# maniacs-oss/shadow

Hardware: AMD Instinct MI355X
Metric: routing-table build GTEPS + packet-routes/sec at 1/2/4/8 MI355X (%HBM roofline) (higher is better)
Workload: dtype f64

## Files before the change

### shadow_amd/csrc/topo_build.cpp

```cpp
#include <dlfcn.h>

#include <cstdio>
#include <cstdlib>
#include <cstring>
#include <numeric>

#include "topo_host.h"

namespace shdtopo {

constexpr int64_t kTieProbeRows = 64;

int upload_layout(Topology* top, const std::vector<uint32_t>& src, const std::vector<uint32_t>& perm,
                  const std::vector<uint32_t>* bstart, double delta, hipStream_t st) {
    const int64_t rows = (int64_t)src.size();
    std::vector<uint32_t>& psrc = top->layPsrc;
    psrc.resize((size_t)rows);
    for (int64_t i = 0; i < rows; i++) psrc[(size_t)i] = src[(size_t)perm[(size_t)i]];
    HIPCHK(top->d_rowmap.ensure((size_t)rows));
    HIPCHK(top->d_bsrc.ensure((size_t)rows));
    HIPCHK(hipMemcpyAsync(top->d_rowmap.p, perm.data(), 4 * (size_t)rows, hipMemcpyHostToDevice, st));
    HIPCHK(hipMemcpyAsync(top->d_bsrc.p, psrc.data(), 4 * (size_t)rows, hipMemcpyHostToDevice, st));
    const std::vector<double> sh = source_shifts(top, psrc.data(), rows, delta);
    HIPCHK(top->d_srcsh.ensure((size_t)rows));
// ... 271 lines not shown
    }
    HIPCHK(hipEventRecord(top->ev0, st));
    HIPCHK(launch_pair_table_complete((int)A, c.row0, c.rows, top->d_elatAA.p, top->d_elossAA.p,
                                      top->d_vlossA.p, c.out_lr, c.out_hops, c.out_rowmin,
                                      top->d_stats.p, st));
    HIPCHK(hipEventRecord(top->ev1, st));
    return 0;
}

int upload_endpoints(Topology* top, RowsCall& c) {
    const int64_t rows = c.rows, A = c.A;
    c.src.resize((size_t)rows);
    c.tgt.resize((size_t)A);
    for (int64_t i = 0; i < rows; i++) c.src[(size_t)i] = (uint32_t)top->hp->inv[(size_t)top->attached[(size_t)(c.row0 + i)]];
    for (int64_t i = 0; i < A; i++) c.tgt[(size_t)i] = (uint32_t)top->hp->inv[(size_t)top->attached[(size_t)i]];
    HIPCHK(top->d_sources.ensure((size_t)rows));
    HIPCHK(top->d_targets.ensure((size_t)A));
    HIPCHK(hipMemcpyAsync(top->d_sources.p, c.src.data(), sizeof(uint32_t) * (size_t)rows, hipMemcpyHostToDevice, c.st));
    HIPCHK(hipMemcpyAsync(top->d_targets.p, c.tgt.data(), sizeof(uint32_t) * (size_t)A, hipMemcpyHostToDevice, c.st));
    c.K = batch_k(top);
    top->stats.peeled_targets = 0;
    HIPCHK(hipEventRecord(top->ev0, c.st));
    return 0;
}

int prepare_target_set(Topology* top, RowsCall& c) {
    hipStream_t st = c.st;
    const int64_t nadjk = (int64_t)(top->d_adjk.n / 4);
    const bool leaf = leaf_targets_on(top);
    if (leaf) {
        CHK(ensure_leaf_targets(top, c.tgt, top->d_targets.p, st));
        c.ws.tleaf = top->d_tleaf.p;
    }
    top->stats.peeled_targets = leaf ? top->leafPeeled : 0;
    if (!top->adjkPlain && (top->adjkTargets != c.tgt || top->adjkLeaf != leaf)) {
        HIPCHK(launch_kappa_copy(top->g.V, nadjk, hub_segs(top), top->d_rowptr.p, adj_out(top), top->d_pot.p,
                                 top->d_sptPar.p, top->d_adjk.p, top->d_kap.p,
                                 top->d_ksum.p, top->d_kap0.p, st));
        top->adjkPlain = true;
        top->adjkFlagged = false;
        top->adjkResorted = false;
        top->adjkLeaf = false;
        top->adjkTargets.clear();
    }
    if (!top->targetSkip || !top->adjkPlain) return 0;
    CHK(upload_target_bits(top, c.tgt, st));
    HIPCHK(hipEventRecord(top->evp0, st));
    const uint32_t* tbits = leaf ? top->d_tbitsEff.p : top->d_tbits.p;
    const uint32_t* dead = leaf ? top->d_dead.p : nullptr;
    HIPCHK(launch_mark_targets(top->d_adjk.p, nadjk, tbits, st));
    const int64_t V = top->g.V;
    const HubSegs hs = hub_segs(top);
    const int nit = std::max(0, top->targetKappa);
    HIPCHK(top->d_kfA.ensure(2 * (size_t)V));
    HIPCHK(top->d_kfB.ensure(2 * (size_t)V));
    HIPCHK(top->d_kfPart.ensure(std::max<size_t>(1, hs.nseg)));
    HIPCHK(top->d_kfChanged.ensure((size_t)nit + 1));
    if (!top->kfKapReady) {
        HIPCHK(top->d_kfKap.ensure((size_t)std::max<int64_t>(1, nadjk)));
        HIPCHK(launch_kfix_kap(adj_out(top), top->d_pot.p, nadjk, top->d_kfKap.p, st));
        top->kfKapReady = true;
    }
    HIPCHK(hipMemsetAsync(top->d_kfChanged.p, 0, sizeof(unsigned int) * ((size_t)nit + 1), st));
    HIPCHK(launch_kfix_step(top->d_rowptr.p, adj_out(top), top->d_kfKap.p, tbits,
                            nullptr, top->d_kfA.p, V, hs, top->d_kfPart.p,
                            top->d_kfChanged.p, st, dead));
// ... 856 lines not shown
```

### shadow_amd/csrc/topo_core.cpp

```cpp
#include <arpa/inet.h>

#include <condition_variable>
#include <cstdarg>
#include <cstdio>
#include <cstdlib>
#include <cstring>
#include <numeric>
#include <queue>
#include <unordered_set>

#include "topo_host.h"

extern "C" {
__attribute__((weak)) uint32_t address_toNetworkIP(Address* address);
__attribute__((weak)) double random_nextDouble(Random* random);
__attribute__((weak)) void worker_updateMinTimeJump(double minPathLatency);
__attribute__((weak)) void logging_log(const char* log_domain, int log_level, const char* fileName,
                                       const char* functionName, int lineNumber,
                                       const char* format, ...);
}
using namespace shdtopo;

namespace shdtopo {
namespace {
// ... 439 lines not shown
        hin.rows = H;
        hin.seg = iseg.p;
        hin.nseg = ns;
        hin.multi = imulti.p;
        hin.nmulti = nm;
        double pm = 0.0;
        HIPCHK(prep_tree(V, nadj, hin, top->d_rowptrIn.p, top->d_adj.p, top->d_aloss.p, top->d_pot.p,
                         top->d_sptPar.p, top->d_spt.p, &pm, st, kTreeParents));
        DevBuf<double> prev;
        HIPCHK(prev.ensure((size_t)V));
        int it2 = 0;
        HIPCHK(prep_h0_distances(V, top->d_rowptrIn.p, top->d_adj.p, prev.p, &it2, st));
        top->hp->potSrc.resize((size_t)V);
        HIPCHK(hipMemcpyAsync(top->hp->potSrc.data(), prev.p, 8 * (size_t)V, hipMemcpyDeviceToHost, st));
        HIPCHK(hipStreamSynchronize(st));
        double mx = 0.0;
        for (double x : top->hp->potSrc)
            if (std::isfinite(x) && x > mx) mx = x;
        top->hp->srcMax = mx;
    }
    step_done(4);
    HIPCHK(top->d_adjk.ensure(4 * (size_t)std::max<int64_t>(1, nadj)));
    HIPCHK(top->d_kap.ensure((size_t)std::max<int64_t>(1, nadj)));
    HIPCHK(top->d_ksum.ensure(kKProbes * (size_t)V));
    HIPCHK(top->d_kap0.ensure((size_t)V));
    HIPCHK(launch_kappa_copy(V, nadj, hub_segs(top), top->d_rowptr.p, adj_out(top), top->d_pot.p,
                             top->d_sptPar.p, top->d_adjk.p, top->d_kap.p, top->d_ksum.p,
                             top->d_kap0.p, st));
    top->adjkPlain = true;
    top->adjkFlagged = false;
    top->adjkLeaf = false;
    top->adjkTargets.clear();
    top->leafFor.clear();
    top->rowsSorted = true;
    HIPCHK(top->d_kfKap.ensure((size_t)std::max<int64_t>(1, nadj)));
    HIPCHK(launch_kfix_kap(adj_out(top), top->d_pot.p, nadj, top->d_kfKap.p, st));
    top->kfKapReady = true;
    step_done(5);
    {
        const auto tc = clk::now();
        top->hp->perm.resize((size_t)V);
        top->hp->inv.resize((size_t)V);
        top->hp->pot.resize((size_t)V);
        top->hp->sptPar.resize((size_t)V);
        HIPCHK(hipMemcpyAsync(top->hp->perm.data(), dperm.p, 4 * (size_t)V, hipMemcpyDeviceToHost, st));
        HIPCHK(hipMemcpyAsync(top->hp->inv.data(), dinv.p, 4 * (size_t)V, hipMemcpyDeviceToHost, st));
        HIPCHK(hipMemcpyAsync(top->hp->pot.data(), top->d_pot.p, 8 * (size_t)V, hipMemcpyDeviceToHost, st));
        HIPCHK(hipMemcpyAsync(top->hp->sptPar.data(), top->d_sptPar.p, 4 * (size_t)V, hipMemcpyDeviceToHost, st));
        HIPCHK(hipStreamSynchronize(st));
        copy_ms += ms_since(tc);
        const auto th = clk::now();
        tree_order(*top->hp);
        host_ms += ms_since(th);
    }
    step_done(6);
    MESSAGE("graph preparation: upload %.1f, relabel %.1f, rows %.1f, h0 distances %.1f (%d "
            "rounds), tree %.1f, kappa copy %.1f, host copies %.1f ms",
            top->stats.csr_step_ms[0], top->stats.csr_step_ms[1], top->stats.csr_step_ms[2],
            top->stats.csr_step_ms[3], iters, top->stats.csr_step_ms[4],
            top->stats.csr_step_ms[5], top->stats.csr_step_ms[6]);
    top->stats.csr_host_ms = host_ms;
    top->stats.csr_copy_ms = copy_ms;
    top->csrUploaded = true;
    return 0;
}

// ... 250 lines not shown
    std::vector<uint32_t> tb(words, 0u);
    for (uint32_t t : tgt) tb[t >> 5] |= 1u << (t & 31u);
    HIPCHK(top->d_tbits.ensure(words));
    HIPCHK(hipMemcpyAsync(top->d_tbits.p, tb.data(), 4 * words, hipMemcpyHostToDevice, st));
    HIPCHK(hipStreamSynchronize(st));
    return 0;
}

bool leaf_targets_on(const Topology* top) { return top->leafTargets && !top->isDirected; }

int ensure_leaf_targets(Topology* top, const std::vector<uint32_t>& tgt, const uint32_t* d_tgt,
                        hipStream_t st) {
    if (top->leafFor == tgt && top->d_tleaf.p) return 0;
    const size_t words = ((size_t)top->g.V + 31) / 32;
    const size_t A = tgt.size();
    std::vector<uint32_t> tb(words, 0u);
    for (uint32_t t : tgt) tb[t >> 5] |= 1u << (t & 31u);
    top->leafFor.clear();
    HIPCHK(top->d_tleaf.ensure(2 * std::max<size_t>(1, A)));
    HIPCHK(top->d_tbitsEff.ensure(words));
    HIPCHK(top->d_dead.ensure(words));
    HIPCHK(top->d_leafCount.ensure(1));
    HIPCHK(hipMemcpyAsync(top->d_tbitsEff.p, tb.data(), 4 * words, hipMemcpyHostToDevice, st));
    HIPCHK(hipMemsetAsync(top->d_dead.p, 0, 4 * words, st));
    HIPCHK(hipMemsetAsync(top->d_leafCount.p, 0, 4, st));
    HIPCHK(launch_leaf_targets(top->d_rowptr.p, top->d_adj.p, top->d_aloss.p, d_tgt, (int)A,
                               top->d_tleaf.p, top->d_tbitsEff.p, top->d_dead.p,
                               top->d_leafCount.p, st));
    uint32_t n = 0;
    HIPCHK(hipMemcpyAsync(&n, top->d_leafCount.p, 4, hipMemcpyDeviceToHost, st));
    HIPCHK(hipStreamSynchronize(st));
    top->leafPeeled = (int64_t)n;
    top->leafFor = tgt;
    return 0;
}

uint64_t compute_geometry(Topology* top) {
    std::vector<int32_t> vs;
    uint64_t sg;
    {
        std::shared_lock<std::shared_mutex> lk(top->ipMu);
        sg = top->setGen.load();
        if (top->geomInit && top->geomGen == top->ipGen) return sg;
        top->geomGen = top->ipGen;
        std::vector<int32_t> def(top->deferredOff.begin(), top->deferredOff.end());
        std::sort(def.begin(), def.end());
        vs.reserve(std::max<size_t>(top->A, 16));
        size_t k = 0;
        const uint32_t* on = top->hostsOn.data();
        for (int32_t v = 0; v < top->g.V; v++) {
            while (k < def.size() && def[k] < v) k++;
            if (on[v] || (k < def.size() && def[k] == v)) vs.push_back(v);
        }
    }
    if (top->geomInit && vs == top->attached) return sg;
    top->geomInit = true;
    top->attached = vs;
    top->A = (int64_t)vs.size();
    top->colOf.assign((size_t)top->g.V, -1);
    for (size_t i = 0; i < vs.size(); i++) top->colOf[(size_t)vs[i]] = (int32_t)i;
    top->colOfShared.reset();
    top->tableValid.store(false);
    if (top->isComplete) {
        auto pb = std::make_unique<Topology::PairBits>();
        pb->words = (size_t)((top->A * top->A + 63) / 64);
        pb->bits.reset(new std::atomic<uint64_t>[std::max<size_t>(1, pb->words)]);
// ... 518 lines not shown
            r = ensure_kprime_scratch(top, nullptr);
        if (!r) r = hipStreamSynchronize(top->stream) == hipSuccess ? 0 : -1;
        step(3);
        top->prepBgRc = r;
        top->prepBgMs = std::chrono::duration<double, std::milli>(std::chrono::steady_clock::now() - t0).count();
        if (onLoad) top->deviceUsed = used;
    });
}

void release_prepared(Topology* top) {
    release_workspace(top);
    for (auto* b : {&top->d_spt, &top->d_sptPar, &top->d_inv, &top->d_rowptr, &top->d_adj,
                    &top->d_adjo, &top->d_rowptrIn, &top->d_adjk})
        b->release();
    for (auto* b : {&top->d_elat, &top->d_eloss, &top->d_aloss, &top->d_vloss, &top->d_selfLat,
                    &top->d_selfLoss, &top->d_pot, &top->d_kfA, &top->d_kfB, &top->d_kfPart,
                    &top->d_kfKap})
        b->release();
    top->kfKapReady = false;
    top->kfFinal = nullptr;
    top->d_eu.release(); top->d_ev.release();
    top->d_kap.release(); top->d_ksum.release(); top->d_kap0.release();
    top->d_hseg.release(); top->d_hmulti.release(); top->d_kfChanged.release();
    top->d_kpKey.release(); top->d_kpIdx.release();
    top->d_kpRec.release(); top->d_kpTmp.release();
    top->d_kpBigPos.release(); top->d_kpBigRow.release(); top->d_kpBigVal.release();
    top->d_kpBigKey.release();
    top->kpBig = -1;
    top->hsegRows = top->hsegN = top->hmultiN = 0;
    top->csrUploaded = top->rowsSorted = false;
    top->adjkPlain = top->adjkFlagged = top->adjkResorted = top->adjkLeaf = false;
    top->adjkTargets.clear();
    top->leafFor.clear();
    top->ordUploaded = false;
    top->ordHp = nullptr;
    top->hp.reset();
}

void do_attach(Topology* top, uint32_t ip, int32_t v, uint64_t* bwDownOut, uint64_t* bwUpOut) {
    if (!top->firstAttachSet.load(std::memory_order_relaxed)) {
        std::unique_lock<std::shared_mutex> lk(top->ipMu);
        if (!top->firstAttachSet.load()) {
            top->firstAttachT = std::chrono::steady_clock::now();
            top->firstAttachSet.store(true);
        }
    }
    start_graph_prep(top, false);
    {
        std::unique_lock<std::shared_mutex> lk(top->ipMu);
        auto it = top->virtualIP.find(ip);
        const int32_t old = it == top->virtualIP.end() ? -1 : it->second;
        top->virtualIP[ip] = v;
        ip_tab_set(top, ip, v);
        top->ipGen++;
        if (old != v) {
            if (old >= 0) host_off(top, old);
            if (v >= 0) host_on(top, v);
        }
    }
    if (v >= 0) {
        if (bwUpOut) *bwUpOut = (uint64_t)top->g.vbwup[(size_t)v];
        if (bwDownOut) *bwDownOut = (uint64_t)top->g.vbwdown[(size_t)v];
    }
}

void do_detach(Topology* top, uint32_t ip) {
// ... 844 lines not shown
        const char* name;
        const void* host;
        const void* dev;
        size_t bytes;
        bool ok;
    };
    const Arr arrs[] = {
        {"perm", hp.perm.data(), nullptr, 4 * V, true},
        {"inv", hp.inv.data(), nullptr, 4 * V, true},
        {"rowptr", nullptr, top->d_rowptr.p, 4 * (V + 1), true},
        {"adj", nullptr, top->d_adj.p, 16 * nadj, true},
        {"aloss", nullptr, top->d_aloss.p, 8 * nadj, true},
        {"vloss", nullptr, top->d_vloss.p, 8 * V, true},
        {"self_lat", nullptr, top->d_selfLat.p, 8 * V, true},
        {"self_loss", nullptr, top->d_selfLoss.p, 8 * V, true},
        {"pot", hp.pot.data(), nullptr, 8 * V, true},
        {"pi_max", &hp.piMax, nullptr, 8, true},
        {"spt_parent", nullptr, top->d_sptPar.p, 4 * V, true},
        {"spt", nullptr, top->d_spt.p, 32 * V, true},
        {"adjk", nullptr, top->d_adjk.p, 16 * nadj, true},
        {"kap", nullptr, top->d_kap.p, 4 * nadj, true},
        {"ksum", nullptr, top->d_ksum.p, 4 * (size_t)kKProbes * V, true},
        {"kap0", nullptr, top->d_kap0.p, 4 * V, true},
        {"kf_kap", nullptr, top->d_kfKap.p, 8 * nadj, top->kfKapReady},
        {"hub_seg", nullptr, top->d_hseg.p, sizeof(uint2) * (size_t)top->hsegN, true},
        {"hub_multi", nullptr, top->d_hmulti.p, sizeof(uint4) * (size_t)top->hmultiN, true},
        {"rowptr_in", nullptr, top->d_rowptrIn.p, 4 * (V + 1), dir},
        {"adj_out", nullptr, top->d_adjo.p, 16 * nadj, dir},
        {"pot_src", hp.potSrc.data(), nullptr, 8 * V, dir && hp.potSrc.size() == V},
        {"tbits", nullptr, top->d_tbits.p, 4 * words, top->adjkFlagged && top->d_tbits.p},
        {"tbits_eff", nullptr, top->d_tbitsEff.p, 4 * words, leaf},
        {"dead", nullptr, top->d_dead.p, 4 * words, leaf},
        {"tleaf", nullptr, top->d_tleaf.p, 32 * top->leafFor.size(), leaf},
        {"kfix", nullptr, top->kfFinal, 16 * V, tprep},
        {"state", state, nullptr, sizeof state, true},
    };
    for (const Arr& a : arrs) {
        if (strcmp(a.name, name) != 0) continue;
        if (!a.ok) return -2;
        if (!out) return (int64_t)a.bytes;
        if (cap_bytes < (int64_t)a.bytes) return -3;
        if (a.bytes == 0) return 0;
        if (a.host) memcpy(out, a.host, a.bytes);
        else if (a.dev) HIPCHK(hipMemcpy(out, a.dev, a.bytes, hipMemcpyDeviceToHost));
        else return -2;
        return (int64_t)a.bytes;
    }
    return -1;
}

int shdtopo_export_graph(Topology* top, int32_t* eu, int32_t* ev, double* elat, double* eloss,
                         double* vloss) {
    if (!top) return -1;
    const HostGraph& g = top->g;
    const size_t E = (size_t)g.E, V = (size_t)g.V;
    if (eu) memcpy(eu, g.eu.data(), 4 * E);
    if (ev) memcpy(ev, g.ev.data(), 4 * E);
    if (elat) memcpy(elat, g.elat.data(), 8 * E);
    if (eloss) memcpy(eloss, g.eloss.data(), 8 * E);
    if (vloss) memcpy(vloss, g.vloss.data(), 8 * V);
    return 0;
}

int shdtopo_write_graphml(Topology* top, const char* path) {
    if (!top || !path) return -1;
    return graphml_write_file(top->g, path) ? 0 : -1;
// ... 295 lines not shown
```

### shadow_amd/csrc/topo_device.h

```cpp
#pragma once

#include <hip/hip_runtime.h>

#include <cstdint>
#include <vector>

namespace shdtopo {

#ifndef SHD_SSSP_BLOCK
#define SHD_SSSP_BLOCK 1024
#endif
constexpr int kSsspBlock = SHD_SSSP_BLOCK;
#ifndef SHD_BATCH_WGPCU
#define SHD_BATCH_WGPCU 1
#endif
constexpr int kBatchWgPerCu = SHD_BATCH_WGPCU;
constexpr int kMaxHops = 48;
constexpr size_t kPathBufPerSlot = (size_t)kMaxHops * kSsspBlock;
constexpr uint32_t kRowScanCap = 16384;
constexpr uint32_t kRsUnreq = 0xFFFFFFFEu;
#ifndef SHD_KAP_IN_REC
#define SHD_KAP_IN_REC 1
#endif
constexpr bool kKapInRec = SHD_KAP_IN_REC != 0;
// ... 55 lines not shown
    const double* aloss = nullptr;
    const double* vloss = nullptr;
    const double* selfLat = nullptr;
    const double* selfLoss = nullptr;
    int rows_sorted = 0;
    int tflags = 0;
    int directed = 0;
    const uint32_t* rowptr_in = nullptr;
};

struct SlotWs {
    int slots = 0;
    int64_t V = 0;
    unsigned long long* dist = nullptr;
    uint4* prec = nullptr;
    unsigned long long* qa = nullptr;
    unsigned long long* qb = nullptr;
    uint32_t* ring = nullptr;
    uint4* rscan = nullptr;
    uint32_t rs_chunk = kRowScanCap;
    double* pathbuf = nullptr;
    uint32_t* counters = nullptr;
    int K = 8;
    int64_t q_stride = 0;
    int64_t ring_entries = 0;
    uint8_t* mask = nullptr;
    uint32_t* hpar = nullptr;
    uint8_t* rowflag = nullptr;
    const uint32_t* rowmap = nullptr;
    unsigned long long* btrace = nullptr;
    const uint32_t* bstart = nullptr;
    int nbat = 0;
    const uint4* tleaf = nullptr;
};
constexpr uint32_t kNoLeaf = 0xFFFFFFFFu;
constexpr int kBTraceWords = 12;

struct ReplayCSR {
    int32_t V = 0;
    int64_t nadj = 0;
    const uint32_t* rowptr = nullptr;
    const uint4* rec = nullptr;
    const uint32_t* own = nullptr;
    const double2* hop = nullptr;
    const double* vloss = nullptr;
    const double* selfLat = nullptr;
    const double* selfLoss = nullptr;
    const uint32_t* tbits = nullptr;
    int64_t ntargets = 0;
    int32_t landmark = -1;
    int32_t intKeys = 0;
};

struct ReplayWs {
    int slots = 0;
    uint4* vrec = nullptr;
    uint4* node = nullptr;
    uint32_t* pathbuf = nullptr;
    uint32_t nodeCap = 0;
    uint32_t stdPos = 0;
    uint32_t stdBase = 0;
};
struct ReplayLayout {
    uint32_t stdPos, stdBase, nodeCap;
};
ReplayLayout replay_layout(int int_keys, uint32_t V);

constexpr uint32_t kHubSeg = 4096;
struct HubSegs {
    uint32_t rows = 0;
    const uint2* seg = nullptr;
    uint32_t nseg = 0;
    const uint4* multi = nullptr;
    uint32_t nmulti = 0;
};
void hub_segments(const uint32_t* rowptr_head, uint32_t rows, std::vector<uint2>& seg,
                  std::vector<uint4>& multi);

struct SsspLdsPlan {
    uint32_t H = 0;
    uint32_t P = 0;
    size_t bytes = 0;
};

SsspLdsPlan sssp_batch_lds_plan(int K, int64_t hub_limit, uint32_t par_hubs, int64_t V);
hipError_t launch_mark_targets(uint32_t* adjk, int64_t nadj, const uint32_t* tbits,
                               hipStream_t stream);
hipError_t launch_kfix_kap(const uint32_t* adj, const double* pot, int64_t nadj, double* kap,
                           hipStream_t stream);
hipError_t launch_kfix_step(const uint32_t* rowptr, const uint32_t* adj, const double* kap_e,
                            const uint32_t* tbits, const double* Kin, double* Kout, int64_t V,
                            const HubSegs& hs, double* part, unsigned int* changed,
                            hipStream_t stream, const uint32_t* dead = nullptr);
hipError_t launch_leaf_targets(const uint32_t* rowptr, const uint32_t* adj, const double* aloss,
                               const uint32_t* targets, int A, uint4* tleaf, uint32_t* tbits,
                               uint32_t* dead, uint32_t* count, hipStream_t stream);
hipError_t launch_kfix_store(uint32_t* adjk, int64_t nadj, const double* K, hipStream_t stream);
constexpr uint32_t kSegBlock = 4096;
struct SegBig {
    const uint32_t* pos = nullptr;
    const uint32_t* row = nullptr;
    int64_t nitems = 0;
    int end_bit = 33;
    unsigned long long* keys = nullptr;
    uint32_t* vals = nullptr;
    void* tmp = nullptr;
    size_t tmp_bytes = 0;
};
struct KprimeScratch {
    float* key = nullptr;
    uint32_t* idx = nullptr;
    uint4* rec = nullptr;
    SegBig big;
};
hipError_t segsort_big_tmp_bytes(int64_t nitems, int end_bit, size_t* bytes);
hipError_t launch_segsort(const uint32_t* rowptr, int64_t V, int64_t nadj, const float* key,
                          float* key_out, uint32_t* idx_out, const SegBig& big, hipStream_t stream);
hipError_t segsort_reference(const uint32_t* rowptr, int64_t V, int64_t nadj, const float* key,
                             const uint32_t* idx_in, float* key_out, uint32_t* idx_out, void* tmp,
                             size_t* tmp_bytes, hipStream_t stream);
hipError_t preload_kprime_sort(hipStream_t stream);
hipError_t launch_kprime_resort(uint32_t* adjk, float* kap, float* ksum, float* kap0,
                                const uint32_t* rowptr, int64_t V, int64_t nadj, const double* pot,
                                const uint32_t* tbits, const double* K, const KprimeScratch& sc,
                                hipStream_t stream);
hipError_t launch_sssp_batch(int K, const DevCSR& g, const SlotWs& ws, const uint32_t* d_sources,
                             const double* d_srcsh, const double* d_h0seed, int nsrc, int kf,
                             const uint32_t* d_targets, int A,
                             double delta, const SsspLdsPlan& plan, uint32_t iter_guard,
// ... 306 lines not shown
```

### shadow_amd/csrc/topo_flows.cpp

```cpp
#include <cstddef>
#include <cstdio>
#include <cstring>

#include "topo_host.h"

namespace shdtopo {

static_assert(sizeof(ShdRoute) == 32 && sizeof(TraceRoute) == sizeof(ShdRoute) &&
                  offsetof(ShdRoute, hops) == offsetof(TraceRoute, hops) &&
                  offsetof(ShdRoute, status) == offsetof(TraceRoute, status) &&
                  offsetof(ShdRoute, latency) == offsetof(TraceRoute, latency) &&
                  offsetof(ShdRoute, reliability) == offsetof(TraceRoute, reliability),
              "TraceRoute is the device image of ShdRoute");

ShdRoute route_blank(int status) { return ShdRoute{-1, -1, status, -1.0, -1.0}; }

int64_t place_routes_host(ShdRoute* routes, int64_t n, int64_t cap) {
    int64_t off = 0;
    for (int64_t i = 0; i < n; i++) {
        if (routes[i].status != kTraceOk) continue;
        const int64_t need = (int64_t)routes[i].hops + 1;
        if (off + need <= cap) {
            routes[i].offset = off;
        } else {
// ... 110 lines not shown
    if (top->slots <= 0 || top->wsK != K || top->wsRing != ring_entries(top, K) ||
        top->wsHpar < hparN || top->wsRsChunk != top->rsChunk) {
        if (ensure_workspace(top, R.nsrc) != 0) {
            (void)hipGetLastError();
            return 0;
        }
        R.keep->stats.slots = top->stats.slots;
        R.keep->stats.workspace_bytes = top->stats.workspace_bytes;
        R.keep->stats.workspace_ms = top->stats.workspace_ms;
    }
    if (top->slots <= 0) return 0;
    R.K = K;
    const int fill = (int)top->stats.batch_fill;
    R.kf = fill >= 1 && fill <= K ? fill : K;
    R.delta = default_delta(top);
    R.plan = batch_lds_plan(top, K);
    R.bcsr = dev_csr(top);
    R.bws = slot_ws(top);
    R.pc = PairChains{R.bws.prec, R.bws.counters, R.bws.slots, K, R.kf};
    const int64_t A = (int64_t)tgt.size();
    const std::vector<double> sh = source_shifts(top, R.srcs.data(), R.nsrc, R.delta);
    HIPCHK(R.d_tgt.ensure((size_t)std::max<int64_t>(1, A)));
    HIPCHK(R.d_srcsh.ensure((size_t)R.nsrc));
    HIPCHK(R.d_bst.ensure(ST_COUNT));
    HIPCHK(hipMemcpy(R.d_tgt.p, tgt.data(), 4 * (size_t)A, hipMemcpyHostToDevice));
    HIPCHK(hipMemcpy(R.d_srcsh.p, sh.data(), 8 * (size_t)R.nsrc, hipMemcpyHostToDevice));
    const std::vector<double> hs = source_h0_seeds(top, R.srcs.data(), R.nsrc);
    HIPCHK(R.d_h0seed.ensure((size_t)R.nsrc));
    HIPCHK(hipMemcpy(R.d_h0seed.p, hs.data(), 8 * (size_t)R.nsrc, hipMemcpyHostToDevice));
    if (leaf) {
        CHK(ensure_leaf_targets(top, tgt, R.d_tgt.p, top->stream));
        R.bws.tleaf = top->d_tleaf.p;
    }
    R.batchOk = true;
    return 0;
}

int group_replay_requests(Topology* top, const std::vector<int32_t>& sv,
                          const std::vector<int32_t>& dv, int64_t n, double* ids_ms,
                          bool forLoadTree, ReplayReqs& R) {
    CHK(dev_init(top));
    CHK(collect_row_stats(top));
    R.keep.reset(new TraceKeep(top));
    CHK(upload_csr(top));
    CHK(upload_replay(top));
    CHK(ensure_trace_ids(top, ids_ms));
    hipStream_t st = top->stream;
    const std::vector<int32_t>& inv = top->hp->inv;

    std::vector<uint32_t>& order = R.order;
    for (int64_t i = 0; i < n; i++)
        if (sv[(size_t)i] >= 0 && dv[(size_t)i] >= 0) order.push_back((uint32_t)i);
    std::stable_sort(order.begin(), order.end(), [&](uint32_t a, uint32_t b) {
        return inv[(size_t)sv[a]] < inv[(size_t)sv[b]];
    });
    const size_t nv = R.nv = order.size();
    std::vector<uint32_t>& srcs = R.srcs;
    std::vector<uint32_t>& srcStart = R.srcStart;
    std::vector<uint32_t> rsi(nv), rsrc(nv), rdst(nv);
    for (size_t q = 0; q < nv; q++) {
        const uint32_t s = (uint32_t)inv[(size_t)sv[order[q]]];
        if (srcs.empty() || srcs.back() != s) {
            srcs.push_back(s);
            srcStart.push_back((uint32_t)q);
        }
        rsi[q] = (uint32_t)srcs.size() - 1u;
// ... 872 lines not shown
```

### shadow_amd/csrc/topo_host.h

```cpp
#pragma once

#include <hip/hip_runtime.h>
#include <rccl/rccl.h>

#include <algorithm>
#include <array>
#include <chrono>
#include <cmath>
#include <deque>
#include <functional>
#include <thread>

#include "../../include/shd_topology_abi.h"
#include "topo_internal.h"

namespace shdtopo {

constexpr int kLogCritical = 1 << 3, kLogWarning = 1 << 4, kLogMessage = 1 << 5, kLogInfo = 1 << 6;

void shd_log(int glevel, const char* file, const char* func, int line, const char* fmt, ...);
#define CRITICAL(...) shd_log(kLogCritical, __FILE__, __FUNCTION__, __LINE__, __VA_ARGS__)
#define WARNING(...) shd_log(kLogWarning, __FILE__, __FUNCTION__, __LINE__, __VA_ARGS__)
#define MESSAGE(...) shd_log(kLogMessage, __FILE__, __FUNCTION__, __LINE__, __VA_ARGS__)
#define INFO(...) shd_log(kLogInfo, __FILE__, __FUNCTION__, __LINE__, __VA_ARGS__)
// ... 167 lines not shown
    DevBuf<double> d_h0seed;
    DevBuf<uint8_t> d_mask;
    DevBuf<uint32_t> d_hpar;
    DevBuf<unsigned long long> d_stats;
    DevBuf<int32_t> b_src, b_dst;
    DevBuf<uint32_t> b_pay, b_sin, b_sout;
    DevBuf<uint64_t> b_now, b_time;
    DevBuf<uint8_t> b_dl;

    bool tieReplay = true;
    bool replayAll = false;
    int tieDenseOpt = -1;
    bool tieDense = false;
    bool tieProbed = false;
    DevBuf<uint32_t> d_probeSrc;
    DevBuf<double> d_probeSh;
    DevBuf<double> d_probeSeed;
    int replaySlotsOpt = 0;
    int replayWpc = 20;
    bool rwsInt = false;
    bool replayLandmark = true;
    bool replayIntOpt = true;
    bool replayIntOk = false;
    int sourceOrder = 2;
    int batchFill = 0;
    int batchOrder = 5;
    bool targetSkip = true;
    std::vector<uint32_t> adjkTargets;
    bool leafTargets = true;
    bool adjkLeaf = false;
    bool h0Seed = true;
    std::vector<uint32_t> leafFor;
    int64_t leafPeeled = 0;
    bool adjkFlagged = false;
    bool adjkPlain = false;
    bool adjkResorted = false;
    bool targetResort = true;
    int targetKappa = 6;
    DevBuf<double> d_pot, d_kfA, d_kfB, d_kfPart;
    DevBuf<double> d_kfKap;
    const double* kfFinal = nullptr;
    bool kfKapReady = false;
    DevBuf<float> d_kpKey;
    DevBuf<uint32_t> d_kpIdx;
    DevBuf<uint4> d_kpRec;
    DevBuf<uint8_t> d_kpTmp;
    DevBuf<uint32_t> d_kpBigPos, d_kpBigRow, d_kpBigVal;
    DevBuf<unsigned long long> d_kpBigKey;
    int64_t kpBig = -1;
    int kpBigBits = 33;
    bool tpPending = false;
    hipEvent_t evp0 = nullptr, evp1 = nullptr;
    DevBuf<uint2> d_hseg;
    DevBuf<uint4> d_hmulti;
    uint32_t hsegRows = 0, hsegN = 0, hmultiN = 0;
    int slotsUsed = 0;
    DevBuf<unsigned int> d_kfChanged;
    DevBuf<uint32_t> d_rowmap, d_bsrc;
    std::vector<uint32_t> ordSrc;
    std::vector<uint32_t> ordBase;
    std::vector<uint32_t> ordPerm;
    bool ordUploaded = false;
    const HostPrep* ordHp = nullptr;
    int balance = 1;
    int64_t lastBatches = 0;
    std::vector<float> srcCost;
    const HostPrep* costHp = nullptr;
    double costA = 0.0;
    std::vector<uint32_t> layPsrc;
    DevBuf<uint32_t> d_bstart;
    DevBuf<unsigned long long> d_btrace;
    int ordKf = -1, ordSO = -1, ordBO = -1;
    double ordDelta = -1.0;
    double ordPhase = -2.0;
    double h0Phase = 0.99;
    bool h0PhaseSet = false;
    bool replayUploaded = false;
    int64_t rnadj = 0;
    DevBuf<uint32_t> d_rrow;
    DevBuf<uint4> d_rrec;
    DevBuf<uint32_t> d_rown;
    DevBuf<double2> d_rhop;
    DevBuf<uint32_t> d_tbits;
    DevBuf<uint4> d_tleaf;
    DevBuf<uint32_t> d_tbitsEff, d_dead, d_leafCount;
    DevBuf<uint4> d_rvrec, d_rnode;
    DevBuf<uint32_t> d_rpath, d_rrows;
    DevBuf<uint8_t> d_rowflag;
    int rslots = 0;
    int rslotsUse = 0;
    hipEvent_t evr0 = nullptr, evr1 = nullptr;
    bool replayPending = false;

    int traceChunk = 0;
    int traceBatch = 1;
    bool traceIdsReady = false;
    DevBuf<int32_t> d_tperm, d_reid, d_selfEid;
    ShdTraceStats traceStats{};
    int loadWalk = 1;
    ShdLoadStats loadStats{};
    ShdCrossStats crossStats{};
    ShdTimelineStats timelineStats{};
    std::vector<std::pair<int, LinkMonitor*>> monitors;
    double monitorIndexMb = 0.0;

    int devicesOpt = 1;
    int xchgMode = 0;
    hipStream_t xstream = nullptr;
    static constexpr int kCopyStreams = 16;
    hipStream_t cstream[kCopyStreams] = {};
    int memShareDiv = 1;
    bool forceRccl = false;
    std::vector<Topology*> peers;
    std::vector<ncclComm_t> comms;
    std::vector<int> commDevs;
    int64_t shardRows = 0;

    std::shared_ptr<const HostTable> snap;
// ... 40 lines not shown
int enqueue_rows(Topology* top, int64_t row0, int64_t row1, double2* out_lr, uint16_t* out_hops,
                 double* out_rowmin, hipStream_t st);
int collect_row_stats(Topology* top);
int build_multi(Topology* top);
int num_devices();
void bstep_mark(Topology* top, int i);
void reset_build_stats(Topology* top);
void plan_long_rows(const uint32_t* rowptr, int64_t V, std::vector<uint32_t>& pos,
                    std::vector<uint32_t>& row, int* end_bit);
int ensure_kprime_scratch(Topology* top, KprimeScratch* out);
__attribute__((visibility("hidden"))) bool layout_from_costs(
    const std::vector<double>& c, double a, int kf, int slots, int K, std::vector<uint32_t>& order,
    std::vector<uint32_t>& lstart);
__attribute__((visibility("hidden"))) void release_comms(Topology* top);

int dev_init(Topology* top);
uint64_t compute_geometry(Topology* top);
int32_t vertex_of_ip(Topology* top, uint32_t ip);
void edge_scan(Topology* top);
Topology* slot_engine(Topology* top, int d);
HubSegs hub_segs(Topology* top);
const uint32_t* adj_out(Topology* top);
void release_workspace(Topology* top);
double h0_phase(Topology* top, double delta);
int upload_csr(Topology* top);
int upload_replay(Topology* top);
int ensure_replay_ws(Topology* top, int nrows);
int upload_target_bits(Topology* top, const std::vector<uint32_t>& tgt, hipStream_t st);
int ensure_workspace(Topology* top, int nsrc);
int hub_rows_ready(Topology* top, uint32_t H, hipStream_t st);
int ensure_leaf_targets(Topology* top, const std::vector<uint32_t>& tgt, const uint32_t* d_tgt,
                        hipStream_t st);
bool leaf_targets_on(const Topology* top);
int batch_k(Topology* top);
int64_t ring_entries(Topology* top, int K);
double default_delta(Topology* top);
SsspLdsPlan batch_lds_plan(Topology* top, int K);
DevCSR dev_csr(Topology* top);
SlotWs slot_ws(Topology* top);
ReplayCSR replay_csr(Topology* top);
ReplayWs replay_ws(Topology* top);
std::vector<double> source_shifts(Topology* top, const uint32_t* s, int64_t n, double delta);
std::vector<double> source_h0_seeds(Topology* top, const uint32_t* s, int64_t n);
bool table_current(Topology* top);
const double2* tab_lr(const Topology* top);
const uint16_t* tab_hops(const Topology* top);
int ensure_table(Topology* top);

template <class S>
int copy_stats(Topology* top, S _Topology::*field, S* out) {
    if (!top || !out) return -1;
    std::lock_guard<std::mutex> lk(top->buildMu);
    *out = top->*field;
    return 0;
}

void monitors_release(Topology* top);


inline uint64_t lat_ns(double ms) { return (uint64_t)std::ceil(ms * 1000000.0); }

inline int bin_add(uint64_t t0, uint64_t binNs, int64_t nbins, uint64_t* bins, uint64_t* outside,
                   int64_t row, uint64_t t, uint64_t w) {
    if (t < t0) {
        if (outside) outside[2 * row] += w;
        return 0;
// ... 161 lines not shown
```

### shadow_amd/csrc/topo_sssp_batch.hip

```cpp
#include <hip/hip_runtime.h>
#include <hipcub/hipcub.hpp>

#include <algorithm>
#include <cmath>
#include <cstddef>
#include <cstdint>
#include <type_traits>

#include "topo_dev_common.h"

namespace shdtopo {

namespace {

using namespace dev;

constexpr int kBatchRB = 2;
constexpr int kBatchU = 2;
constexpr int kBChunk = 512;
#ifndef SHD_BATCH_WRCOUNT
#define SHD_BATCH_WRCOUNT 0
#endif
#ifndef SHD_BATCH_TIME
#define SHD_BATCH_TIME 0
// ... 840 lines not shown
            const uint32_t* P = list ? qb : qa;
            uint32_t* const S = fscr;
            const uint32_t pcapS = (uint32_t)(V * K);
            const bool gs = kind == kJobWalkSync;
            auto put = [&](uint32_t q, uint32_t u, double loss) {
                const unsigned long long lb = d2bits(loss);
                wl_count(L, WL_PREC, true, precO + q);
                precO[q] = make_uint4(u, eptv, (uint32_t)lb, (uint32_t)(lb >> 32));
            };
            auto load_hop = [&](uint32_t v, uint32_t j) -> Hop {
                Hop hh;
                const uint32_t q = v * K + j;
                rl_count(L, RL_WALK, v >= H, reinterpret_cast<const uint4*>(g.spt) + 2 * (size_t)v);
                rl_count(L, RL_WALK, true, distO + (size_t)q);
                if (v >= H) {
                    const uint4* sp = reinterpret_cast<const uint4*>(g.spt) + 2 * (size_t)v;
                    hh.sp = sp[0];
                    const uint2 l = *reinterpret_cast<const uint2*>(sp + 1);
                    hh.sl = __hiloint2double((int)l.y, (int)l.x);
                } else {
                    hh.sp = make_uint4(0xFFFFFFFFu, 0u, 0u, 0u);
                    hh.sl = 0.0;
                }
                hh.d = ld_l2_u64(&distO[(size_t)q]);
                return hh;
            };
            uint32_t i = 0, iend = 0, q = 0, j = 0;
            uint32_t nw = 0, nw0 = 0;
            bool act = false, fresh = false, more = true;
            Hop h;
            h.sp = make_uint4(0xFFFFFFFFu, 0u, 0u, 0u);
            h.sl = 0.0;
            h.d = 0ull;
            for (;;) {
                if (more && !__any(i < iend)) {
                    uint32_t c;
                    const uint32_t b = grab(&c);
                    if (b == kJobNone) {
                        more = false;
                    } else {
                        i = b + lane;
                        iend = b + c;
                    }
                }
                bool take = !act && i < iend;
                if (gs) {
                    const unsigned long long am = __ballot(act);
                    take = take && ((am >> (lane & ~(uint32_t)(K - 1))) & ((1ull << K) - 1ull)) == 0ull;
                }
                rl_count(L, RL_WALK, take, P + (take ? i : 0u));
                if (take) {
                    q = P[i];
                    i += 64;
                    j = q % K;
                    act = q != kNoPair;
                    fresh = act;
                }
                if (!more && !__any(act || i < iend)) break;
                bool sp = false;
                if (act && fresh) {
                    h = load_hop(q / K, j);
                    fresh = false;
                } else if (act) {
                    const uint32_t v = q / K;
                    const uint32_t pu = h.sp.x;
                    const bool tree = v >= H && pu < (uint32_t)V;
                    Hop hn = h;
                    if (tree) hn = load_hop(pu, j);
                    rl_count(L, RL_WALK, true, precwO + 4 * (size_t)q);
                    const uint32_t tw = ld_l2_u32(&precwO[4 * (size_t)q + 1]);
                    if (tag_claimed(tw, epv)) {
                        act = false;
                    } else {
                        nw++;
                        const bool tied = tag_tied(tw, epv);
                        if (tree && !tied &&
                            __dadd_rn(bits2d(hn.d), __hiloint2double((int)h.sp.w, (int)h.sp.z)) ==
                                bits2d(h.d)) {
                            put(q, pu, h.sl);
                            nw0++;
                            if (pu == L.src[j]) {
                                act = false;
                            } else {
                                q = pu * K + j;
                                h = hn;
                            }
                        } else {
                            wl_count(L, WL_PREC, true, precwO + 4 * (size_t)q);
                            precwO[4 * (size_t)q + 1] = eptv | (tied ? kTagTie : 0u);
                            sp = true;
// ... 40 lines not shown
                        rl_count(L, RL_EPI, true, ws.tleaf + 2 * (size_t)k);
                        const uint4 la = ws.tleaf[2 * (size_t)k];
                        const uint2 lb = *reinterpret_cast<const uint2*>(ws.tleaf + 2 * (size_t)k + 1);
                        t = la.x;
                        lu = la.y;
                        lw = __hiloint2double((int)la.w, (int)la.z);
                        ll = __hiloint2double((int)lb.y, (int)lb.x);
                    } else {
                        rl_count(L, RL_EPI, true, targets + k);
                        t = targets[k];
                    }
                    const uint32_t src = L.src[jj];
                    double lat, rel;
                    uint32_t hcnt = 0;
                    if (t == src) {
                        const double sl = g.selfLat[src];
                        if (isnan(sl)) {
                            atomicAdd(&stats[ST_ERRORS], 1ull);
                            lat = -1.0;
                            rel = -1.0;
                        } else {
                            lat = 0.0 + sl;
                            rel = 1.0;
                            rel *= (1.0 - g.vloss[src]);
                            rel *= (1.0 - g.selfLoss[src]);
                            hcnt = 1;
                        }
                    } else {
                        const bool leaf = lu != kNoLeaf;
                        const uint32_t v0 = leaf ? lu : t;
                        rl_count(L, RL_EPI, true, distO + (size_t)v0 * K + jj);
                        rl_count(L, RL_EPI, true, g.vloss + t);
                        lat = bits2d(ld_l2_u64(&distO[(size_t)v0 * K + jj]));
                        bool amb = false, bad = false;
                        uint32_t v = v0;
                        if (leaf) {
                            lat = __dadd_rn(lat, lw);
                            *pb_at(0u) = ll;
                            hcnt = 1;
                            if (KEEP) {
                                const unsigned long long lb = d2bits(ll);
                                wl_count(L, WL_PREC, true, precO + (size_t)t * K + jj);
                                precO[(size_t)t * K + jj] =
                                    make_uint4(lu, eptv, (uint32_t)lb, (uint32_t)(lb >> 32));
                            }
                        }
                        while (v != src) {
                            typedef unsigned int u32x4 __attribute__((ext_vector_type(4)));
                            rl_count(L, RL_EPI, true, reinterpret_cast<const u32x4*>(precO) + (size_t)v * K + jj);
                            const u32x4 rv = __builtin_nontemporal_load(
                                reinterpret_cast<const u32x4*>(precO) + (size_t)v * K + jj);
                            if (rv.y != eptv || (rv.x & 0x40000000u)) {
                                bad = true;
                                break;
                            }
                            amb |= (rv.x >> 31) != 0u;
                            wl_count(L, WL_OTHER, hcnt < kMaxHops && hcnt >= nl, pb_at(hcnt));
                            if (hcnt < kMaxHops) *pb_at(hcnt) = __hiloint2double((int)rv.w, (int)rv.z);
                            hcnt++;
                            v = rv.x & 0x3FFFFFFFu;
                            if (hcnt > (uint32_t)V) { bad = true; break; }
                        }
                        rel = 1.0;
                        rel *= (1.0 - g.vloss[src]);
                        rel *= (1.0 - g.vloss[t]);
                        if (bad) {
                            atomicAdd(&stats[ST_ERRORS], 1ull);
                            lat = -1.0;
                            rel = -1.0;
                        } else if (hcnt <= (uint32_t)kMaxHops) {
                            for (int x = (int)hcnt - 1; x >= 0; --x) rel *= (1.0 - *pb_at((uint32_t)x));
                        } else {
                            atomicAdd(&stats[ST_LONGPATH], 1ull);
                            for (int x = (int)hcnt - 1; x >= 0; --x) {
                                if (leaf && x == 0) {
                                    rel *= (1.0 - ll);
                                    continue;
                                }
                                uint32_t y = v0;
                                for (int z = leaf ? 1 : 0; z < x; ++z) y = precO[(size_t)y * K + jj].x & 0x3FFFFFFFu;
                                const uint4 r = precO[(size_t)y * K + jj];
                                rel *= (1.0 - __hiloint2double((int)r.w, (int)r.z));
                            }
                        }
                        if (amb) {
                            atomicAdd(&stats[ST_AMBIGUOUS], 1ull);
                            if (ws.rowflag) ws.rowflag[ws.rowmap ? ws.rowmap[r0v + jj] : r0v + jj] = 1;
                        }
                        if (lat == 0.0) lat = 1.0;
                    }
                    const size_t ob = (size_t)(ws.rowmap ? (int)ws.rowmap[r0v + jj] : (int)(r0v + jj)) * (size_t)A + k;
                    const uint16_t hh = (uint16_t)(hcnt > 65535u ? 65535u : hcnt);
                    wl_count(L, WL_OUT, !KEEP, out_lr + ob);
                    wl_count(L, WL_OUT, !KEEP, out_hops + ob);
                    if (!KEEP) {
                        typedef double f64x2 __attribute__((ext_vector_type(2)));
                        const f64x2 r2 = {lat, rel};
                        __builtin_nontemporal_store(r2, reinterpret_cast<f64x2*>(out_lr) + ob);
// ... 805 lines not shown
                                    uint4* __restrict__ tleaf, uint32_t* __restrict__ tbits,
                                    uint32_t* __restrict__ dead, uint32_t* __restrict__ count) {
    const int k = (int)(blockIdx.x * blockDim.x + threadIdx.x);
    if (k >= A) return;
    const uint32_t t = targets[k];
    const uint32_t r0 = rowptr[t], r1 = rowptr[t + 1];
    uint4 a = make_uint4(t, kNoLeaf, 0u, 0u), b = make_uint4(0u, 0u, 0u, 0u);
    if (r1 - r0 == 1u) {
        const AdjRec r = *reinterpret_cast<const AdjRec*>(adj + kAdjWords * r0);
        const uint32_t u = r.a;
        if (u != t && rowptr[u + 1] - rowptr[u] > 1u) {
            const unsigned long long lb = d2bits(aloss[r0]);
            a = make_uint4(t, u, r.b, r.c);
            b = make_uint4((uint32_t)lb, (uint32_t)(lb >> 32), 0u, 0u);
            atomicAnd(&tbits[t >> 5], ~(1u << (t & 31u)));
            atomicOr(&tbits[u >> 5], 1u << (u & 31u));
            atomicOr(&dead[t >> 5], 1u << (t & 31u));
            atomicAdd(count, 1u);
        }
    }
    tleaf[2 * (size_t)k] = a;
    tleaf[2 * (size_t)k + 1] = b;
}

hipError_t launch_leaf_targets(const uint32_t* rowptr, const uint32_t* adj, const double* aloss,
                               const uint32_t* targets, int A, uint4* tleaf, uint32_t* tbits,
                               uint32_t* dead, uint32_t* count, hipStream_t stream) {
    if (A <= 0) return hipSuccess;
    hipLaunchKernelGGL(leaf_targets_kernel, dim3((unsigned)((A + 255) / 256)), dim3(256), 0, stream,
                       rowptr, adj, aloss, targets, A, tleaf, tbits, dead, count);
    return hipGetLastError();
}

__global__ void kfix_kap_kernel(const uint32_t* __restrict__ adj, const double* __restrict__ pot,
                                int64_t nadj, double* __restrict__ kap) {
    for (int64_t k = (int64_t)blockIdx.x * blockDim.x + threadIdx.x; k < nadj;
         k += (int64_t)gridDim.x * blockDim.x) {
        const uint32_t y = adj[kAdjWords * k];
        const double w = __hiloint2double((int)adj[kAdjWords * k + 3], (int)adj[kAdjWords * k + 2]);
        const double p = pot[y];
        kap[k] = isfinite(p) ? w - p : -INFINITY;
    }
}

__device__ __forceinline__ double kfix_term(const uint32_t* adj, const double* kap_e,
                                            const double* Ktin, uint32_t k) {
    const double kap = kap_e[k];
    double t = kap;
    if (Ktin) {
        const uint32_t y = adj[kAdjWords * k];
        const double w = __hiloint2double((int)adj[kAdjWords * k + 3], (int)adj[kAdjWords * k + 2]);
        const double ky = Ktin[y] + w * (1.0 - 2e-5) - 1e-9;
        t = ky > kap ? ky : kap;
    }
    return t;
}

__device__ __forceinline__ double kfix_dead(const uint32_t* dead, uint32_t x, double m) {
    return dead && ((dead[x >> 5] >> (x & 31u)) & 1u) ? INFINITY : m;
}
__device__ __forceinline__ void kfix_put(double* Kout, double* Ktout, const uint32_t* tbits,
                                         uint32_t x, double m) {
    Kout[x] = m;
    Ktout[x] = ((tbits[x >> 5] >> (x & 31u)) & 1u) ? -INFINITY : m;
}

// ... 519 lines not shown
```

### shadow_amd/topology.py

```python
from __future__ import annotations

import ctypes
import socket
import struct

import numpy as np

from . import _lib as L


def ip_to_network(ip: str) -> int:
    return struct.unpack("<I", socket.inet_aton(ip))[0]


def network_to_ip(n: int) -> str:
    return socket.inet_ntoa(struct.pack("<I", n & 0xFFFFFFFF))


class Address:

    def __init__(self, ip):
        lib, shim = L.load()
        self.ip = ip_to_network(ip) if isinstance(ip, str) else int(ip)
        self._p = shim.shim_address_new(self.ip)
# ... 245 lines not shown
        ev = np.empty(E, np.int32)
        el = np.empty(E, np.float64)
        lo = np.empty(E, np.float64)
        vl = np.empty(V, np.float64)
        if self._lib.shdtopo_export_graph(self._h, _p(eu), _p(ev), _p(el), _p(lo), _p(vl)) != 0:
            raise RuntimeError("export_graph failed")
        return V, eu, ev, el, lo, vl

    def export_csr(self):
        n = int(self._lib.shdtopo_export_csr(self._h, None, None, None, None, None))
        if n < 0:
            raise RuntimeError("shdtopo_export_csr failed: %d" % n)
        V = self.num_vertices
        perm = np.empty(V, np.int32)
        rowptr = np.empty(V + 1, np.uint32)
        col = np.empty(max(n, 1), np.uint32)
        pot = np.empty(V, np.float64)
        par = np.empty(V, np.uint32)
        r = self._lib.shdtopo_export_csr(self._h, _p(perm), _p(rowptr), _p(col), _p(pot), _p(par))
        if r != n:
            raise RuntimeError("shdtopo_export_csr failed: %d" % r)
        return dict(perm=perm, rowptr=rowptr, col=col[:n], pot=pot, tree_parent=par)

    PREP_ARRAYS = {
        "perm": (np.int32, ()), "inv": (np.int32, ()), "rowptr": (np.uint32, ()),
        "adj": (np.uint32, (4,)), "aloss": (np.float64, ()), "vloss": (np.float64, ()),
        "self_lat": (np.float64, ()), "self_loss": (np.float64, ()), "pot": (np.float64, ()),
        "pi_max": (np.float64, ()), "spt_parent": (np.uint32, ()), "spt": (np.uint32, (8,)),
        "adjk": (np.uint32, (4,)), "kap": (np.float32, ()), "ksum": (np.float32, None),
        "kap0": (np.float32, ()), "kf_kap": (np.float64, ()), "hub_seg": (np.uint32, (2,)),
        "hub_multi": (np.uint32, (4,)), "rowptr_in": (np.uint32, ()),
        "adj_out": (np.uint32, (4,)), "pot_src": (np.float64, ()), "tbits": (np.uint32, ()),
        "tbits_eff": (np.uint32, ()), "dead": (np.uint32, ()), "tleaf": (np.uint32, (8,)),
        "kfix": (np.float64, ()), "state": (np.int32, ()),
    }
    PREP_STATE = ("adjk_plain", "flagged", "resorted", "leaf", "kprobes", "kap_in_rec",
                  "hub_seg_len", "group_hubs")

    def export_prep(self, names=None):
        out = {}
        for name in (names if names is not None else self.PREP_ARRAYS):
            dt, shape = self.PREP_ARRAYS[name]
            n = int(self._lib.shdtopo_export_prep(self._h, name.encode(), None, 0))
            if n == -2 and names is None:
                continue
            if n == -2:
                raise KeyError(name)
            if n < 0:
                raise RuntimeError("shdtopo_export_prep(%s) failed: %d" % (name, n))
            buf = np.empty(max(n, 1), np.uint8)
            r = int(self._lib.shdtopo_export_prep(self._h, name.encode(), _p(buf), n))
            if r != n:
                raise RuntimeError("shdtopo_export_prep(%s) failed: %d" % (name, r))
            out[name] = buf[:n].view(dt)
        if "state" in out:
            out["state"] = dict(zip(self.PREP_STATE, (int(x) for x in out["state"])))
        for name, a in out.items():
            if name == "state":
                continue
            shape = self.PREP_ARRAYS[name][1]
            if shape is None:
                a = a.reshape(self.num_vertices, -1)
            elif shape:
                a = a.reshape((-1,) + shape)
            out[name] = a
        return out

# ... 456 lines not shown
```

Baseline: 2660.

## Precompute per-target walk start records and prefetch next pair in route walk

Adds a kernel that gathers each target's shortest-path-tree start record (following leaf peeling when active) into a compact per-target table, cached across calls with the same target set. The route-walk loop now prefetches the next pair index and its start record one iteration ahead, and seeds walker state directly from that table instead of running the fresh-start path. It also hoists the two vloss loads earlier in the epilogue. The aim is to hide walk-start load latency and skip redundant start work, at the cost of an extra buffer, a cached host vector and more live registers in the walk kernel.

```diff
diff --git a/shadow_amd/csrc/topo_build.cpp b/shadow_amd/csrc/topo_build.cpp
--- a/shadow_amd/csrc/topo_build.cpp
+++ b/shadow_amd/csrc/topo_build.cpp
@@ -327,6 +327,8 @@
         CHK(ensure_leaf_targets(top, c.tgt, top->d_targets.p, st));
         c.ws.tleaf = top->d_tleaf.p;
     }
+    CHK(ensure_walk_starts(top, c.tgt, top->d_targets.p, leaf, st));
+    c.ws.tstart = top->d_tstart.p;
     top->stats.peeled_targets = leaf ? top->leafPeeled : 0;
     if (!top->adjkPlain && (top->adjkTargets != c.tgt || top->adjkLeaf != leaf)) {
         HIPCHK(launch_kappa_copy(top->g.V, nadjk, hub_segs(top), top->d_rowptr.p, adj_out(top), top->d_pot.p,
diff --git a/shadow_amd/csrc/topo_core.cpp b/shadow_amd/csrc/topo_core.cpp
--- a/shadow_amd/csrc/topo_core.cpp
+++ b/shadow_amd/csrc/topo_core.cpp
@@ -495,6 +495,7 @@
     top->adjkLeaf = false;
     top->adjkTargets.clear();
     top->leafFor.clear();
+    top->startFor.clear();
     top->rowsSorted = true;
     HIPCHK(top->d_kfKap.ensure((size_t)std::max<int64_t>(1, nadj)));
     HIPCHK(launch_kfix_kap(adj_out(top), top->d_pot.p, nadj, top->d_kfKap.p, st));
@@ -811,6 +812,19 @@
     HIPCHK(hipStreamSynchronize(st));
     top->leafPeeled = (int64_t)n;
     top->leafFor = tgt;
+    return 0;
+}
+
+int ensure_walk_starts(Topology* top, const std::vector<uint32_t>& tgt, const uint32_t* d_tgt,
+                       bool leaf, hipStream_t st) {
+    if (top->startFor == tgt && top->startLeaf == leaf && top->d_tstart.p) return 0;
+    const size_t A = tgt.size();
+    top->startFor.clear();
+    HIPCHK(top->d_tstart.ensure(2 * std::max<size_t>(1, A)));
+    HIPCHK(launch_walk_starts(top->d_spt.p, d_tgt, leaf ? top->d_tleaf.p : nullptr, (int)A,
+                              top->d_tstart.p, st));
+    top->startFor = tgt;
+    top->startLeaf = leaf;
     return 0;
 }
 
@@ -1395,6 +1409,7 @@
     top->adjkPlain = top->adjkFlagged = top->adjkResorted = top->adjkLeaf = false;
     top->adjkTargets.clear();
     top->leafFor.clear();
+    top->startFor.clear();
     top->ordUploaded = false;
     top->ordHp = nullptr;
     top->hp.reset();
@@ -2305,6 +2320,8 @@
         {"tbits_eff", nullptr, top->d_tbitsEff.p, 4 * words, leaf},
         {"dead", nullptr, top->d_dead.p, 4 * words, leaf},
         {"tleaf", nullptr, top->d_tleaf.p, 32 * top->leafFor.size(), leaf},
+        {"tstart", nullptr, top->d_tstart.p, 32 * top->startFor.size(),
+         top->d_tstart.p && !top->startFor.empty()},
         {"kfix", nullptr, top->kfFinal, 16 * V, tprep},
         {"state", state, nullptr, sizeof state, true},
     };
diff --git a/shadow_amd/csrc/topo_device.h b/shadow_amd/csrc/topo_device.h
--- a/shadow_amd/csrc/topo_device.h
+++ b/shadow_amd/csrc/topo_device.h
@@ -111,6 +111,7 @@
     const uint32_t* bstart = nullptr;
     int nbat = 0;
     const uint4* tleaf = nullptr;
+    const uint4* tstart = nullptr;
 };
 constexpr uint32_t kNoLeaf = 0xFFFFFFFFu;
 constexpr int kBTraceWords = 12;
@@ -174,6 +175,8 @@
 hipError_t launch_leaf_targets(const uint32_t* rowptr, const uint32_t* adj, const double* aloss,
                                const uint32_t* targets, int A, uint4* tleaf, uint32_t* tbits,
                                uint32_t* dead, uint32_t* count, hipStream_t stream);
+hipError_t launch_walk_starts(const uint32_t* spt, const uint32_t* targets, const uint4* tleaf,
+                              int A, uint4* tstart, hipStream_t stream);
 hipError_t launch_kfix_store(uint32_t* adjk, int64_t nadj, const double* K, hipStream_t stream);
 constexpr uint32_t kSegBlock = 4096;
 struct SegBig {
diff --git a/shadow_amd/csrc/topo_flows.cpp b/shadow_amd/csrc/topo_flows.cpp
--- a/shadow_amd/csrc/topo_flows.cpp
+++ b/shadow_amd/csrc/topo_flows.cpp
@@ -166,6 +166,8 @@
         CHK(ensure_leaf_targets(top, tgt, R.d_tgt.p, top->stream));
         R.bws.tleaf = top->d_tleaf.p;
     }
+    CHK(ensure_walk_starts(top, tgt, R.d_tgt.p, leaf, top->stream));
+    R.bws.tstart = top->d_tstart.p;
     R.batchOk = true;
     return 0;
 }
diff --git a/shadow_amd/csrc/topo_host.h b/shadow_amd/csrc/topo_host.h
--- a/shadow_amd/csrc/topo_host.h
+++ b/shadow_amd/csrc/topo_host.h
@@ -223,6 +223,8 @@
     bool h0Seed = true;
     std::vector<uint32_t> leafFor;
     int64_t leafPeeled = 0;
+    std::vector<uint32_t> startFor;
+    bool startLeaf = false;
     bool adjkFlagged = false;
     bool adjkPlain = false;
     bool adjkResorted = false;
@@ -275,6 +277,7 @@
     DevBuf<uint32_t> d_tbits;
     DevBuf<uint4> d_tleaf;
     DevBuf<uint32_t> d_tbitsEff, d_dead, d_leafCount;
+    DevBuf<uint4> d_tstart;
     DevBuf<uint4> d_rvrec, d_rnode;
     DevBuf<uint32_t> d_rpath, d_rrows;
     DevBuf<uint8_t> d_rowflag;
@@ -381,6 +384,8 @@
 int ensure_leaf_targets(Topology* top, const std::vector<uint32_t>& tgt, const uint32_t* d_tgt,
                         hipStream_t st);
 bool leaf_targets_on(const Topology* top);
+int ensure_walk_starts(Topology* top, const std::vector<uint32_t>& tgt, const uint32_t* d_tgt,
+                       bool leaf, hipStream_t st);
 int batch_k(Topology* top);
 int64_t ring_entries(Topology* top, int K);
 double default_delta(Topology* top);
diff --git a/shadow_amd/csrc/topo_sssp_batch.hip b/shadow_amd/csrc/topo_sssp_batch.hip
--- a/shadow_amd/csrc/topo_sssp_batch.hip
+++ b/shadow_amd/csrc/topo_sssp_batch.hip
@@ -896,6 +896,22 @@
             h.sp = make_uint4(0xFFFFFFFFu, 0u, 0u, 0u);
             h.sl = 0.0;
             h.d = 0ull;
+            uint32_t qn = kNoPair;
+            uint4 spn = make_uint4(0xFFFFFFFFu, 0u, 0u, 0u);
+            uint2 sln = make_uint2(0u, 0u);
+            auto fetch_next = [&](bool on) {
+                on = on && i < iend;
+                rl_count(L, RL_WALK, on, P + (on ? i : 0u));
+                rl_count(L, RL_WALK, gs && on, ws.tstart + 2 * (size_t)(on ? i / K : 0u));
+                if (on) {
+                    qn = P[i];
+                    if (gs) {
+                        const uint4* rec = ws.tstart + 2 * (size_t)(i / K);
+                        spn = rec[0];
+                        sln = *reinterpret_cast<const uint2*>(rec + 1);
+                    }
+                }
+            };
             for (;;) {
                 if (more && !__any(i < iend)) {
                     uint32_t c;
@@ -905,6 +921,7 @@
                     } else {
                         i = b + lane;
                         iend = b + c;
+                        fetch_next(true);
                     }
                 }
                 bool take = !act && i < iend;
@@ -912,14 +929,22 @@
                     const unsigned long long am = __ballot(act);
                     take = take && ((am >> (lane & ~(uint32_t)(K - 1))) & ((1ull << K) - 1ull)) == 0ull;
                 }
-                rl_count(L, RL_WALK, take, P + (take ? i : 0u));
                 if (take) {
-                    q = P[i];
+                    q = qn;
                     i += 64;
                     j = q % K;
                     act = q != kNoPair;
-                    fresh = act;
-                }
+                    fresh = act && !gs;
+                }
+                const bool st0 = gs && take && act;
+                rl_count(L, RL_WALK, st0, distO + (st0 ? (size_t)q : (size_t)0));
+                if (st0) {
+                    const bool tail = q / K >= H;
+                    h.sp = tail ? spn : make_uint4(0xFFFFFFFFu, 0u, 0u, 0u);
+                    h.sl = tail ? __hiloint2double((int)sln.y, (int)sln.x) : 0.0;
+                    h.d = ld_l2_u64(&distO[(size_t)q]);
+                }
+                fetch_next(take);
                 if (!more && !__any(act || i < iend)) break;
                 bool sp = false;
                 if (act && fresh) {
@@ -1026,6 +1051,7 @@
                         rl_count(L, RL_EPI, true, distO + (size_t)v0 * K + jj);
                         rl_count(L, RL_EPI, true, g.vloss + t);
                         lat = bits2d(ld_l2_u64(&distO[(size_t)v0 * K + jj]));
+                        const double vls = g.vloss[src], vlt = g.vloss[t];
                         bool amb = false, bad = false;
                         uint32_t v = v0;
                         if (leaf) {
@@ -1056,8 +1082,8 @@
                             if (hcnt > (uint32_t)V) { bad = true; break; }
                         }
                         rel = 1.0;
-                        rel *= (1.0 - g.vloss[src]);
-                        rel *= (1.0 - g.vloss[t]);
+                        rel *= (1.0 - vls);
+                        rel *= (1.0 - vlt);
                         if (bad) {
                             atomicAdd(&stats[ST_ERRORS], 1ull);
                             lat = -1.0;
@@ -1929,6 +1955,30 @@
     return hipGetLastError();
 }
 
+__global__ void walk_starts_kernel(const uint4* __restrict__ spt,
+                                   const uint32_t* __restrict__ targets,
+                                   const uint4* __restrict__ tleaf, int A,
+                                   uint4* __restrict__ tstart) {
+    const int k = (int)(blockIdx.x * blockDim.x + threadIdx.x);
+    if (k >= A) return;
+    uint32_t s = targets[k];
+    if (tleaf) {
+        const uint32_t u = tleaf[2 * (size_t)k].y;
+        if (u != kNoLeaf) s = u;
+    }
+    const uint4 a = spt[2 * (size_t)s], b = spt[2 * (size_t)s + 1];
+    tstart[2 * (size_t)k] = a;
+    tstart[2 * (size_t)k + 1] = make_uint4(b.x, b.y, 0u, 0u);
+}
+
+hipError_t launch_walk_starts(const uint32_t* spt, const uint32_t* targets, const uint4* tleaf,
+                              int A, uint4* tstart, hipStream_t stream) {
+    if (A <= 0) return hipSuccess;
+    hipLaunchKernelGGL(walk_starts_kernel, dim3((unsigned)((A + 255) / 256)), dim3(256), 0, stream,
+                       reinterpret_cast<const uint4*>(spt), targets, tleaf, A, tstart);
+    return hipGetLastError();
+}
+
 __global__ void kfix_kap_kernel(const uint32_t* __restrict__ adj, const double* __restrict__ pot,
                                 int64_t nadj, double* __restrict__ kap) {
     for (int64_t k = (int64_t)blockIdx.x * blockDim.x + threadIdx.x; k < nadj;
diff --git a/shadow_amd/topology.py b/shadow_amd/topology.py
--- a/shadow_amd/topology.py
+++ b/shadow_amd/topology.py
@@ -301,7 +301,7 @@
         "hub_multi": (np.uint32, (4,)), "rowptr_in": (np.uint32, ()),
         "adj_out": (np.uint32, (4,)), "pot_src": (np.float64, ()), "tbits": (np.uint32, ()),
         "tbits_eff": (np.uint32, ()), "dead": (np.uint32, ()), "tleaf": (np.uint32, (8,)),
-        "kfix": (np.float64, ()), "state": (np.int32, ()),
+        "tstart": (np.uint32, (8,)), "kfix": (np.float64, ()), "state": (np.int32, ()),
     }
     PREP_STATE = ("adjk_plain", "flagged", "resorted", "leaf", "kprobes", "kap_in_rec",
                   "hub_seg_len", "group_hubs")
```

Result: faster. 2715, median of 6 (+2.1%).
